# TUI-NICR/EMSANet

Hardware: AMD Instinct MI355X
Metric: images/sec (640x480 RGB-D, bs=32/GPU) fwd+bwd (higher is better)
Workload: dtype f32; 1 GPU; BASELINE.json configs[1]: full EMSANet RGB-D (resnet34-NBt1D x2, SE-add fusion, PPM, semantic+instance+orientation+scene heads), 640x480, bs=32/GPU, f32, train mode (BN batch stats, Dropout2d), step = fwd + bwd (fixed output cotangents) + grad all-reduce + SGD-nesterov update at lr 0 (fixed weights) replayed from a hipGraph; global_batch=32, parallelism=dp1, weights=random init (deterministic), mode=train-hipgraph

## Files before the change

emsanet_amd/csrc/conv_mfma.hip:

```cpp
#include "common.h"

#include <type_traits>
#include <vector>

#include "prof.h"

namespace {

struct ProfSlotImpl {
  hipEvent_t a, b;
  int cls;
  double flops, bytes;
};
std::vector<ProfSlotImpl> g_prof_pool;
size_t g_prof_used = 0;
int g_prof_every = 0;
int g_prof_seen[kProfClasses] = {0};
double g_prof_next_flops = 0.0;
const char* const kProfNames[kProfClasses] = {
    "conv_igemm_kernel<128,128,2,2>", "conv_igemm_kernel<128,64,4,2>",
    "conv_igemm_kernel<64,64,2,2>",   "conv_igemm_kernel<128,32,4,1>",
    "conv_wgrad_kernel<64,32,7,2,1,2>", "conv_wgrad_kernel<128,128,1,2,2,1> (unused)",
    "conv_wgrad_kernel<64,64,1,2,2,1>", "conv_wgrad_kernel<64,64,3,2,2,1>|conv_wgrad1d_wino_kernel<64,64> (1-D convs)",
    "conv1d_wino_kernel (1-D 3x1/1x3 convs)", "conv_h_kernel (16-bit igemm)",
// ... 841 lines not shown

  if (s_begin < s_end) {
    load_regs(s_begin);
    store_lds();
  }
  __syncthreads();

  for (int s = s_begin; s < s_end; ++s) {
    const bool has_next = s + 1 < s_end;
    mleft = mleft_n;
    mright = mright_n;
    if (has_next) load_regs(s + 1);
    const float* d = dS + lh * BCO + wco * 32 + l31;
    const float* x = xS + lh * BCI + wci * 32 + l31;
#pragma unroll
    for (int kk = 0; kk < PK / 2; ++kk) {
      const int r = 2 * kk + lh;
      const float fa = d[kk * 2 * BCO];
      const bool okl = !((mleft >> r) & 1u), okr = !((mright >> r) & 1u);
#pragma unroll
      for (int t = 0; t < 3; ++t) {
        float fb = x[(kk * 2 + t) * BCI];
        if (t == 0) fb = okl ? fb : 0.f;
        if (t == 2) fb = okr ? fb : 0.f;
        acc[0][t] = __builtin_amdgcn_mfma_f32_32x32x2f32(fa, fb, acc[0][t], 0, 0, 0);
      }
    }
    __syncthreads();
    if (has_next) store_lds();
    __syncthreads();
  }

  if (p.ws != nullptr) {
    float* wt = p.ws + (((size_t)ks * p.R + kr) * p.n_tiles + tile) * (3 * BCO * BCI);
#pragma unroll
    for (int t = 0; t < 3; ++t)
#pragma unroll
      for (int r = 0; r < 16; ++r) {
        const int row = (r & 3) + 8 * (r >> 2) + 4 * lh;
        wt[(t * BCO + wco * 32 + row) * BCI + wci * 32 + l31] = acc[0][t][r];
      }
  } else {
#pragma unroll
  for (int t = 0; t < 3; ++t)
#pragma unroll
    for (int q = 0; q < NQ; ++q) {
      const int ci = ci0 + wci * 32 + l31;
#pragma unroll
      for (int r = 0; r < 16; ++r) {
        const int row = (r & 3) + 8 * (r >> 2) + 4 * lh;
        const int co = co0 + wco * 32 + row;
#if EMSA_ABL & 2
        if (co < p.n_ch && ci < p.k_ch && acc[q][t][r] == 1.2345e30f)
#else
        if (co < p.n_ch && ci < p.k_ch)
#endif
          unsafeAtomicAdd(p.dw + ((size_t)(kr * 3 + t) * p.n_ch + co) * p.k_ch + ci, acc[q][t][r]);
      }
    }
  }
  if (do_bias) {
    float* red = smem;
    __syncthreads();
    red[d_r * BCO + d_c4 + 0] = bsum.x;
    red[d_r * BCO + d_c4 + 1] = bsum.y;
    red[d_r * BCO + d_c4 + 2] = bsum.z;
    red[d_r * BCO + d_c4 + 3] = bsum.w;
    __syncthreads();
    if (tid < BCO) {
      float a = 0.f;
      for (int r = 0; r < 256 / DTPR; ++r) a += red[r * BCO + tid];
      if (p.ws_bias != nullptr)
        p.ws_bias[((size_t)ks * p.n_co_tiles + co_t) * BCO + tid] = a;
      else if (co0 + tid < p.n_ch)
        unsafeAtomicAdd(p.dbias + co0 + tid, a);
    }
  }
}

typedef __bf16 gbf16x8 __attribute__((ext_vector_type(8)));
#ifndef EMSA_W1DW_XBN_WPE
#define EMSA_W1DW_XBN_WPE 3
#endif
template <int BCO, int BCI, bool BF16 = false, typename T = float, bool XBN = false>
__global__ __launch_bounds__(256, XBN ? EMSA_W1DW_XBN_WPE : EMSA_W1DW_WPE) void conv_wgrad1d_wino_kernel(const Wgrad1dArgs p) {
  static_assert(BCO == 64 && BCI == 64, "wave layout below is for a 64x64 (co x ci) tile");
  static_assert(!XBN || (!BF16 && sizeof(T) == 4), "the folded input BatchNorm is an fp32 form");
  constexpr uint32_t ES = sizeof(T);
  constexpr int PK = 32, NP = PK / 2, XROWS = PK + 2;
  extern __shared__ __attribute__((aligned(16))) float smem[];
  float* const eS = smem;
  float* const dS = smem + NP * 4 * BCO;
  constexpr int kBL = 20;
  __bf16* const eH = reinterpret_cast<__bf16*>(smem);
  __bf16* const dH = eH + 4 * BCO * kBL;

  const int tid = threadIdx.x, lane = tid & 63, wave = tid >> 6;
  const int l31 = lane & 31, lh = lane >> 5;
  const int wco = wave & 1, wci = wave >> 1;
#if EMSA_W1D_XCD
  const int wg = emsa_xcd_remap(blockIdx.x, gridDim.x);
#else
  const int wg = blockIdx.x;
#endif
  const int tile = wg % p.n_tiles, kr = (wg / p.n_tiles) % p.R;
  const int ks = wg / (p.n_tiles * p.R);
  const int dline = p.R == 3 ? kr - 1 : 0;
  const int ci_t = tile % p.n_ci_tiles, co_t = tile / p.n_ci_tiles;
  const int co0 = co_t * BCO, ci0 = ci_t * BCI;
  const int s_begin = ks * p.steps_per_split;
  const int s_end = min(s_begin + p.steps_per_split, p.steps_total);
  const __amdgpu_buffer_rsrc_t rs_in = make_rsrc(p.in, p.in_bytes);
  const __amdgpu_buffer_rsrc_t rs_dy = make_rsrc(p.dout, p.dout_bytes);
  const int col4 = (tid & 15) * 4, pr = tid >> 4;
  const bool do_bias = p.dbias != nullptr && ci_t == 0 && kr == 0;
  const bool dok = co0 + col4 < p.n_ch, xok = ci0 + col4 < p.k_ch;
  const uint32_t dadd = dok ? (uint32_t)(co0 + col4) * ES : 0u, dmask = dok ? 0u : kOOB;
  const uint32_t xadd = xok ? (uint32_t)(ci0 + col4) * ES : 0u, xmask = xok ? 0u : kOOB;

  typename Raw4<T>::type re_raw[2], rx_raw[4];
  float4 bsum = emsa_zero4();
  uint32_t x_real = 0;
  float* const xbnS = smem + NP * 4 * (BCO + BCI);
  if constexpr (XBN) {
    if (tid < 2 * BCI) {
      const int ch = ci0 + (tid & (BCI - 1));
      const float* src = tid < BCI ? p.in_scale : p.in_shift;
      xbnS[tid] = ch < p.k_ch ? src[ch] : 0.f;
    }
  }
  auto load_regs = [&](int s) {
    const int k = s * PK + lane - 1;
    const bool valid = lane < XROWS && k >= 0 && k < p.M;
    const uint32_t ku = valid ? (uint32_t)k : 0u;
    const uint32_t img = fast_div(ku, p.div_al);
    const uint32_t line = fast_div(ku, p.div_l);
    const int b_ = (int)(ku - __umul24(line, (uint32_t)p.L));
    const int a_ = (int)(line - __umul24(img, (uint32_t)p.A));
    const int a2 = a_ + dline;
    const bool in_line = valid && b_ < p.Lr;
    const uint32_t off_d = in_line
        ? (__umul24(img, (uint32_t)p.dy_simg) + __umul24((uint32_t)a_, (uint32_t)p.dy_sa) +
           __umul24((uint32_t)b_, (uint32_t)p.dy_sb)) * ES : kOOB;
    const uint32_t off_x = (in_line && a2 >= 0 && a2 < p.A)
        ? (__umul24(img, (uint32_t)p.in_simg) + __umul24((uint32_t)a2, (uint32_t)p.in_sa) +
           __umul24((uint32_t)b_, (uint32_t)p.in_sb)) * ES : kOOB;
    const uint32_t off_xl = b_ == p.L - 1 ? kOOB : off_x;
    const uint32_t off_xr = b_ == 0 ? kOOB : off_x;
    const int l0 = (2 * pr) * 4;
    const uint32_t o_e0 = (uint32_t)__builtin_amdgcn_ds_bpermute(l0 + 4, (int)off_d);
    const uint32_t o_e1 = (uint32_t)__builtin_amdgcn_ds_bpermute(l0 + 8, (int)off_d);
    const uint32_t o_d0 = (uint32_t)__builtin_amdgcn_ds_bpermute(l0, (int)off_xl);
    const uint32_t o_d1 = (uint32_t)__builtin_amdgcn_ds_bpermute(l0 + 4, (int)off_x);
    const uint32_t o_d2 = (uint32_t)__builtin_amdgcn_ds_bpermute(l0 + 8, (int)off_x);
    const uint32_t o_d3 = (uint32_t)__builtin_amdgcn_ds_bpermute(l0 + 12, (int)off_xr);
    re_raw[0] = buf_ld4raw<T>(rs_dy, (o_e0 + dadd) | dmask);
    re_raw[1] = buf_ld4raw<T>(rs_dy, (o_e1 + dadd) | dmask);
    rx_raw[0] = buf_ld4raw<T>(rs_in, (o_d0 + xadd) | xmask);
    rx_raw[1] = buf_ld4raw<T>(rs_in, (o_d1 + xadd) | xmask);
    rx_raw[2] = buf_ld4raw<T>(rs_in, (o_d2 + xadd) | xmask);
    rx_raw[3] = buf_ld4raw<T>(rs_in, (o_d3 + xadd) | xmask);
    if constexpr (XBN)
      x_real = (~o_d0 >> 31) | ((~o_d1 >> 31) << 1) | ((~o_d2 >> 31) << 2) | ((~o_d3 >> 31) << 3);
  };
  auto add4 = [](const float4& a, const float4& b) {
    return make_float4(a.x + b.x, a.y + b.y, a.z + b.z, a.w + b.w);
  };
  auto sub4 = [](const float4& a, const float4& b) {
    return make_float4(a.x - b.x, a.y - b.y, a.z - b.z, a.w - b.w);
  };
  auto store_lds = [&]() {
    const float4 re[2] = {raw_f4(re_raw[0], (T*)nullptr), raw_f4(re_raw[1], (T*)nullptr)};
    float4 rx[4] = {raw_f4(rx_raw[0], (T*)nullptr), raw_f4(rx_raw[1], (T*)nullptr),
                    raw_f4(rx_raw[2], (T*)nullptr), raw_f4(rx_raw[3], (T*)nullptr)};
    if constexpr (XBN) {
      typedef float f2 __attribute__((ext_vector_type(2)));
      const float4 sc = emsa_ld4(xbnS + col4), sh = emsa_ld4(xbnS + BCI + col4);
#pragma unroll
      for (int r = 0; r < 4; ++r) {
        const float cap = (x_real >> r) & 1u ? __builtin_inff() : 0.f;
        const f2 lo = __builtin_elementwise_fma(f2{rx[r].x, rx[r].y}, f2{sc.x, sc.y}, f2{sh.x, sh.y});
        const f2 hi = __builtin_elementwise_fma(f2{rx[r].z, rx[r].w}, f2{sc.z, sc.w}, f2{sh.z, sh.w});
        rx[r] = make_float4(__builtin_amdgcn_fmed3f(lo.x, 0.f, cap), __builtin_amdgcn_fmed3f(lo.y, 0.f, cap),
                            __builtin_amdgcn_fmed3f(hi.x, 0.f, cap), __builtin_amdgcn_fmed3f(hi.y, 0.f, cap));
      }
    }
// ... 46 lines not shown
  for (int s = s_begin; s < s_end; ++s) {
#endif
    const bool has_next = s + 1 < s_end;
    if (has_next) load_regs(s + 1);
    if constexpr (BF16) {
#pragma unroll
      for (int c = 0; c < 4; ++c) {
        const uint2* ea = reinterpret_cast<const uint2*>(eH + (c * BCO + wco * 32 + l31) * kBL + 8 * lh);
        const uint2* da = reinterpret_cast<const uint2*>(dH + (c * BCI + wci * 32 + l31) * kBL + 8 * lh);
        const uint2 e0 = ea[0], e1 = ea[1], d0 = da[0], d1 = da[1];
        const uint4 eu = make_uint4(e0.x, e0.y, e1.x, e1.y), du = make_uint4(d0.x, d0.y, d1.x, d1.y);
        acc[c] = __builtin_amdgcn_mfma_f32_32x32x16_bf16(__builtin_bit_cast(gbf16x8, eu),
                                                         __builtin_bit_cast(gbf16x8, du), acc[c],
                                                         0, 0, 0);
      }
    } else {
    const float* e = eS + lh * 4 * BCO + wco * 32 + l31;
    const float* d = dS + lh * 4 * BCI + wci * 32 + l31;
#pragma unroll
    for (int kk = 0; kk < NP / 2; ++kk) {
#pragma unroll
      for (int c = 0; c < 4; ++c)
        acc[c] = __builtin_amdgcn_mfma_f32_32x32x2f32(e[(kk * 8 + c) * BCO], d[(kk * 8 + c) * BCI],
                                                      acc[c], 0, 0, 0);
    }
    }
    __syncthreads();
    if (has_next) store_lds();
    __syncthreads();
  }

#pragma unroll
  for (int r = 0; r < 16; ++r) {
    const float m0 = acc[0][r], m1 = acc[1][r], m2 = acc[2][r], m3 = acc[3][r];
    const float hs = 0.5f * (m1 + m2);
    acc[0][r] = m0 + hs;
    acc[1][r] = 0.5f * (m1 - m2);
    acc[2][r] = hs - m3;
  }

  if (p.ws != nullptr) {
    float* wt = p.ws + (((size_t)ks * p.R + kr) * p.n_tiles + tile) * (3 * BCO * BCI);
#pragma unroll
    for (int t = 0; t < 3; ++t)
#pragma unroll
      for (int r = 0; r < 16; ++r) {
        const int row = (r & 3) + 8 * (r >> 2) + 4 * lh;
        wt[(t * BCO + wco * 32 + row) * BCI + wci * 32 + l31] = acc[t][r];
      }
  } else {
    const int ci = ci0 + wci * 32 + l31;
#pragma unroll
    for (int t = 0; t < 3; ++t)
#pragma unroll
      for (int r = 0; r < 16; ++r) {
        const int row = (r & 3) + 8 * (r >> 2) + 4 * lh;
        const int co = co0 + wco * 32 + row;
#if EMSA_ABL & 2
        if (co < p.n_ch && ci < p.k_ch && acc[t][r] == 1.2345e30f)
#else
        if (co < p.n_ch && ci < p.k_ch)
#endif
          unsafeAtomicAdd(p.dw + ((size_t)(kr * 3 + t) * p.n_ch + co) * p.k_ch + ci, acc[t][r]);
      }
  }
  if (do_bias) {
    float* red = smem;
    __syncthreads();
    red[pr * BCO + col4 + 0] = bsum.x;
    red[pr * BCO + col4 + 1] = bsum.y;
    red[pr * BCO + col4 + 2] = bsum.z;
    red[pr * BCO + col4 + 3] = bsum.w;
    __syncthreads();
    if (tid < BCO) {
      float a = 0.f;
      for (int r = 0; r < NP; ++r) a += red[r * BCO + tid];
      if (p.ws_bias != nullptr)
        p.ws_bias[((size_t)ks * p.n_co_tiles + co_t) * BCO + tid] = a;
      else if (co0 + tid < p.n_ch)
        unsafeAtomicAdd(p.dbias + co0 + tid, a);
    }
  }
}

#ifndef EMSA_WH_DBG
#define EMSA_WH_DBG 0
#endif
#if EMSA_WH_DBG
__device__ long long g_wh_dbg[8 * 4 * 4096];
#define WH_MARK(ph)                                               \
  do {                                                            \
    const long long t_ = (long long)__builtin_readcyclecounter(); \
    dbg_t[ph] += t_ - dbg_prev;                                   \
    dbg_prev = t_;                                                \
  } while (0)
#else
#define WH_MARK(ph) do {} while (0)
#endif
#if defined(__HIP_DEVICE_COMPILE__)
#define EMSA_NO_LSOPT __attribute__((target("no-load-store-opt")))
#else
#define EMSA_NO_LSOPT
#endif
#ifndef EMSA_WH_PK
#define EMSA_WH_PK 64
#endif
constexpr int kWH_PK = EMSA_WH_PK;
constexpr int kWH_NH = kWH_PK / 64;
constexpr int kWH_ROW = kWH_PK + 4;
template <typename T, int MODE = 0>
__global__ __launch_bounds__(256, 3) EMSA_NO_LSOPT void conv_wgrad1d_h_kernel(const Wgrad1dArgs p) {
  constexpr int BCO = 64, BCI = 64;
  constexpr uint32_t ES = sizeof(T);
  constexpr int NT_ = MODE == 1 ? 1 : 3;
  typedef unsigned int u32x4h __attribute__((ext_vector_type(4)));
  extern __shared__ __attribute__((aligned(16))) float smem[];
  T* const dS = reinterpret_cast<T*>(smem);
  T* const xS = dS + BCO * kWH_ROW;
  T* const oS = xS + BCI * kWH_ROW;

  const int tid = threadIdx.x, lane = tid & 63, wave = __builtin_amdgcn_readfirstlane(tid >> 6);
  const int l31 = lane & 31, lh = lane >> 5;
  const int wco = wave & 1, wci = wave >> 1;
#if EMSA_W1D_XCD
  const int wg = emsa_xcd_remap(blockIdx.x, gridDim.x);
#else
  const int wg = blockIdx.x;
#endif
  const int tile = wg % p.n_tiles, kr = (wg / p.n_tiles) % p.R;
  const int ks = wg / (p.n_tiles * p.R);
  const int dline = kr * p.dl_mul + p.dl_off;
  const int ci_t = tile % p.n_ci_tiles, co_t = tile / p.n_ci_tiles;
  const int co0 = co_t * BCO, ci0 = ci_t * BCI;
  const int s_begin = ks * p.steps_per_split;
  const int s_end = min(s_begin + p.steps_per_split, p.steps_total);
  const __amdgpu_buffer_rsrc_t rs_in = make_rsrc(p.in, p.in_bytes);
  const __amdgpu_buffer_rsrc_t rs_dy = make_rsrc(p.dout, p.dout_bytes);
  const int q = (lane & 3) | ((lane >> 4) << 2);
  const int pg = wave * 4 + ((lane >> 2) & 3);
  const bool do_bias = p.dbias != nullptr && ci_t == 0 && kr == 0;
  const bool dok = co0 + 4 * q < p.n_ch, xok = ci0 + 4 * q < p.k_ch;
  const uint32_t dadd = dok ? (uint32_t)(co0 + 4 * q) * ES : 0u, dmask = dok ? 0u : kOOB;
  const uint32_t xadd = xok ? (uint32_t)(ci0 + 4 * q) * ES : 0u, xmask = xok ? 0u : kOOB;

  uint32_t oo_last = kOOB;
  auto px_off = [&](int k, uint32_t& od, uint32_t& ox) {
    const bool valid = k >= 0 && k < p.M;
    const uint32_t ku = valid ? (uint32_t)k : 0u;
    const uint32_t img = fast_div(ku, p.div_al);
    const uint32_t line = fast_div(ku, p.div_l);
    const int b_ = (int)(ku - __umul24(line, (uint32_t)p.L));
    const int a_ = (int)(line - __umul24(img, (uint32_t)p.A));
    const int a2 = a_ * p.x_mul_a + dline;
    const bool in_line = valid && b_ < p.Lr;
    od = in_line ? (__umul24(img, (uint32_t)p.dy_simg) + __umul24((uint32_t)a_, (uint32_t)p.dy_sa) +
                    __umul24((uint32_t)b_, (uint32_t)p.dy_sb)) * ES : kOOB;
    ox = (in_line && a2 >= 0 && a2 < p.in_Ax)
        ? (__umul24(img, (uint32_t)p.in_simg) + __umul24((uint32_t)a2, (uint32_t)p.in_sa1) +
           __umul24((uint32_t)b_, (uint32_t)p.in_sb)) * ES : kOOB;
    if constexpr (MODE == 2)
      oo_last = (ox != kOOB && 2 * b_ + 1 < p.in_Lx) ? ox + (uint32_t)p.in_sb1 * ES : kOOB;
  };

  u32x2w rd[kWH_NH][4], rx[kWH_NH][4], ro[kWH_NH][4];
  u32x2w sv_d = {0u, 0u}, sv_x = {0u, 0u}, sv_o = {0u, 0u};
  float4 bsum = emsa_zero4();
// ... 134 lines not shown
    if constexpr (MODE != 1) prev_s = *reinterpret_cast<const unsigned*>(srow0 + kWH_PK);
    if constexpr (MODE == 0) prev_d = *reinterpret_cast<const unsigned*>(drow0 + kWH_PK);
    __builtin_amdgcn_s_setprio(1);
#pragma unroll
    for (int k16 = 0; k16 < kWH_PK / 16; ++k16) {
      const u32x4h a = ld8(drow, 16 * k16);
      const u32x4h c = ld8(xrow, 16 * k16);
      const ev8 av = __builtin_bit_cast(ev8, a);
      if constexpr (MODE == 1) {
        mma(acc[0], av, c);
      } else if constexpr (MODE == 2) {
        const u32x4h o_ = ld8(srow, 16 * k16);
        const u32x4h lft = shifted(o_, prev_s);
        mma(acc[0], av, lft);
        mma(acc[1], av, c);
        mma(acc[2], av, o_);
      } else {
        const u32x4h lft = shifted(c, prev_s);
        const u32x4h a_sh = shifted(a, prev_d);
        mma(acc[0], av, lft);
        mma(acc[1], av, c);
        mma(acc[2], __builtin_bit_cast(ev8, a_sh), c);
      }
    }
    __builtin_amdgcn_s_setprio(0);
    WH_MARK(1);
    __syncthreads();
    WH_MARK(2);
    if (has_next) store_lds();
    WH_MARK(3);
    __syncthreads();
    WH_MARK(4);
  }

  if (p.ws != nullptr) {
    float* wt = p.ws + (((size_t)ks * p.R + kr) * p.n_tiles + tile) * (NT_ * BCO * BCI);
#pragma unroll
    for (int t = 0; t < NT_; ++t)
#pragma unroll
      for (int r = 0; r < 16; ++r) {
        const int row = (r & 3) + 8 * (r >> 2) + 4 * lh;
        wt[(t * BCO + wco * 32 + row) * BCI + wci * 32 + l31] = acc[t][r];
      }
  } else {
    const int ci = ci0 + wci * 32 + l31;
#pragma unroll
    for (int t = 0; t < NT_; ++t)
#pragma unroll
      for (int r = 0; r < 16; ++r) {
        const int row = (r & 3) + 8 * (r >> 2) + 4 * lh;
        const int co = co0 + wco * 32 + row;
        if (co < p.n_ch && ci < p.k_ch)
          unsafeAtomicAdd(p.dw + ((size_t)(kr * NT_ + t) * p.n_ch + co) * p.k_ch + ci, acc[t][r]);
      }
  }
#if EMSA_WH_DBG
  WH_MARK(6);
  dbg_t[7] = dbg_prev - dbg_t0;
  if (lane == 0 && blockIdx.x < 4096)
    for (int i = 0; i < 8; ++i) g_wh_dbg[(blockIdx.x * 4 + wave) * 8 + i] = dbg_t[i];
#endif
  if (do_bias) {
    float* red = smem;
    __syncthreads();
    red[pg * BCO + 4 * q + 0] = bsum.x;
    red[pg * BCO + 4 * q + 1] = bsum.y;
    red[pg * BCO + 4 * q + 2] = bsum.z;
    red[pg * BCO + 4 * q + 3] = bsum.w;
    __syncthreads();
    if (tid < BCO) {
      float a = 0.f;
      for (int r = 0; r < 16; ++r) a += red[r * BCO + tid];
      if (p.ws_bias != nullptr)
        p.ws_bias[((size_t)ks * p.n_co_tiles + co_t) * BCO + tid] = a;
      else if (co0 + tid < p.n_ch)
        unsafeAtomicAdd(p.dbias + co0 + tid, a);
    }
  }
}

constexpr int kWT_PK = 64;
constexpr int kWT_RS = 96;
constexpr int kWT_IMG = (kWT_PK + 2) * kWT_RS;
constexpr int kWgradMultiMax = 4;
struct WgradMulti {
  Wgrad1dArgs j[kWgradMultiMax];
};

template <typename T, bool XBN = false>
__device__ __forceinline__ void wgrad1d_tr_body(const Wgrad1dArgs& p, const int bid, const int nblk) {
  constexpr int BCO = 64, BCI = 64;
  constexpr uint32_t ES = sizeof(T);
  typedef unsigned int u32x4h __attribute__((ext_vector_type(4)));
  typedef short s16x4 __attribute__((ext_vector_type(4)));
  typedef __attribute__((address_space(3))) s16x4 lds_s16x4;
  extern __shared__ __attribute__((aligned(16))) float smem[];
  T* const dS = reinterpret_cast<T*>(smem);
  T* const xS = dS + kWT_IMG;
  float* const xbnS = reinterpret_cast<float*>(xS + kWT_IMG);

  const int tid = threadIdx.x, lane = tid & 63, wave = __builtin_amdgcn_readfirstlane(tid >> 6);
  const int wco = wave & 1, wci = wave >> 1;
#if EMSA_W1D_XCD
  const int wg = emsa_xcd_remap(bid, nblk);
#else
  const int wg = bid;
#endif
  const int tile = wg % p.n_tiles, kr = (wg / p.n_tiles) % p.R;
  const int ks = wg / (p.n_tiles * p.R);
  const int dline = kr * p.dl_mul + p.dl_off;
  const int ci_t = tile % p.n_ci_tiles, co_t = tile / p.n_ci_tiles;
  const int co0 = co_t * BCO, ci0 = ci_t * BCI;
  const int s_begin = ks * p.steps_per_split;
  const int s_end = min(s_begin + p.steps_per_split, p.steps_total);
  const __amdgpu_buffer_rsrc_t rs_in = make_rsrc(p.in, p.in_bytes);
  const __amdgpu_buffer_rsrc_t rs_dy = make_rsrc(p.dout, p.dout_bytes);
  const int lp = tid >> 2, ch0 = (lane & 3) * 8;
  const bool do_bias = p.dbias != nullptr && ci_t == 0 && kr == 0;
  uint32_t dadd[2], xadd[2];
#pragma unroll
  for (int h = 0; h < 2; ++h) {
    dadd[h] = co0 + ch0 + 32 * h < p.n_ch ? (uint32_t)(co0 + ch0 + 32 * h) * ES : kOOB;
    xadd[h] = ci0 + ch0 + 32 * h < p.k_ch ? (uint32_t)(ci0 + ch0 + 32 * h) * ES : kOOB;
  }
  auto px_off = [&](int k, uint32_t& od, uint32_t& ox) {
    const bool valid = k >= 0 && k < p.M;
    const uint32_t ku = valid ? (uint32_t)k : 0u;
    const uint32_t img = fast_div(ku, p.div_al);
    const uint32_t line = fast_div(ku, p.div_l);
    const int b_ = (int)(ku - __umul24(line, (uint32_t)p.L));
    const int a_ = (int)(line - __umul24(img, (uint32_t)p.A));
    const int a2 = a_ * p.x_mul_a + dline;
    const bool in_line = valid && b_ < p.Lr;
    od = in_line ? (__umul24(img, (uint32_t)p.dy_simg) + __umul24((uint32_t)a_, (uint32_t)p.dy_sa) +
                    __umul24((uint32_t)b_, (uint32_t)p.dy_sb)) * ES : kOOB;
    ox = (in_line && a2 >= 0 && a2 < p.in_Ax)
        ? (__umul24(img, (uint32_t)p.in_simg) + __umul24((uint32_t)a2, (uint32_t)p.in_sa1) +
           __umul24((uint32_t)b_, (uint32_t)p.in_sb)) * ES : kOOB;
  };
  const bool xbn = XBN && p.in_scale != nullptr;
  if constexpr (XBN) {
    if (xbn && tid < 2 * BCI) {
      const int ch = ci0 + (tid & (BCI - 1));
      const float* src = tid < BCI ? p.in_scale : p.in_shift;
      xbnS[tid] = ch < p.k_ch ? src[ch] : 0.f;
    }
  }
  u32x4h rd[2], rx[2];
  [[maybe_unused]] bool x_real = false;
  auto load_px = [&](int k, u32x4h (&d)[2], u32x4h (&x)[2]) {
    uint32_t od, ox;
    px_off(k, od, ox);
    if constexpr (XBN) x_real = ox != kOOB;
#pragma unroll
    for (int h = 0; h < 2; ++h) {
      d[h] = __builtin_amdgcn_raw_buffer_load_b128(rs_dy, (int)(od | dadd[h]) >= 0 ? (int)(od + dadd[h]) : (int)kOOB, 0, 0);
      x[h] = __builtin_amdgcn_raw_buffer_load_b128(rs_in, (int)(ox | xadd[h]) >= 0 ? (int)(ox + xadd[h]) : (int)kOOB, 0, 0);
    }
  };
  float bsum[2][8];
#pragma unroll
  for (int h = 0; h < 2; ++h)
#pragma unroll
    for (int e = 0; e < 8; ++e) bsum[h][e] = 0.f;
  [[maybe_unused]] auto xbn_apply = [&](u32x4h (&x)[2]) {
    if constexpr (XBN) {
      if (xbn) {
        typedef typename std::conditional<std::is_same<T, emsa_f16>::value, _Float16, __bf16>::type EX;
        typedef EX ex8 __attribute__((ext_vector_type(8)));
        typedef float fx8 __attribute__((ext_vector_type(8)));
// ... 692 lines not shown
          } else
            hipLaunchKernelGGL((conv_wgrad1d_tr_kernel<T>), grid, dim3(256),
                               (size_t)2 * kWT_IMG * sizeof(T), st, w);
        } else if (in_scale) {
          prof_end(ps, st);
          return EMSA_E_SHAPE;
        } else
          hipLaunchKernelGGL((conv_wgrad1d_h_kernel<T, 0>), grid, dim3(256),
                             (size_t)2 * 64 * kWH_ROW * sizeof(T), st, w);
      } else if constexpr (!kF16)
      hipLaunchKernelGGL((conv_wgrad1d_wino_kernel<BCO, BCI, true, T>),
                         dim3(w.n_tiles * w.R * pl.ksplit), dim3(256),
                         (size_t)(16 * 4 * (BCO + BCI)) * sizeof(float), st, w);
    } else if (pl.wino && in_scale) {
      if constexpr (!kHalf)
        hipLaunchKernelGGL((conv_wgrad1d_wino_kernel<BCO, BCI, false, float, true>),
                           dim3(w.n_tiles * w.R * pl.ksplit), dim3(256),
                           (size_t)(16 * 4 * (BCO + BCI) + 2 * BCI) * sizeof(float), st, w);
    } else if (in_scale) {
      prof_end(ps, st);
      return EMSA_E_SHAPE;
    } else if (pl.wino && bf16)
      hipLaunchKernelGGL((conv_wgrad1d_wino_kernel<BCO, BCI, true>),
                         dim3(w.n_tiles * w.R * pl.ksplit), dim3(256),
                         (size_t)(16 * 4 * (BCO + BCI)) * sizeof(float), st, w);
    else if (pl.wino)
      hipLaunchKernelGGL((conv_wgrad1d_wino_kernel<BCO, BCI>), dim3(w.n_tiles * w.R * pl.ksplit),
                         dim3(256), (size_t)(16 * 4 * (BCO + BCI)) * sizeof(float), st, w);
    else
      hipLaunchKernelGGL((conv_wgrad1d_kernel<BCO, BCI>), dim3(w.n_tiles * w.R * pl.ksplit),
                         dim3(256), lds, st, w);
    static const bool rows_on = [] {
      const char* e = getenv("EMSA_WGRAD_REDUCE_ROWS");
      return !(e && e[0] == '0');
    }();
    if (ws != nullptr && rows_on && pl.ksplit <= 16 && w.n_tiles >= 32)
      hipLaunchKernelGGL(wgrad1d_reduce_rows_kernel, dim3(w.n_tiles * 4 + w.n_co_tiles),
                         dim3(256), 0, st, ws, w.ws_bias, pl.ksplit, w.n_tiles, w.n_ci_tiles,
                         w.n_co_tiles, w.n_ch, w.k_ch, w.R, dw, dbias, w.taps);
    else if (ws != nullptr)
      hipLaunchKernelGGL(wgrad1d_reduce_kernel, dim3(w.n_tiles * w.R * w.taps * 64 + w.n_co_tiles),
                         dim3(256), 0, st, ws, w.ws_bias, pl.ksplit, w.n_tiles, w.n_ci_tiles,
                         w.n_co_tiles, w.n_ch, w.k_ch, w.R, dw, dbias, w.taps);
    prof_end(ps, st);
    return emsa_launch_status();
  }
  if (in_scale) return EMSA_E_SHAPE;
  if (taps == 7 && g->k_ch <= 32) return launch_wgrad<64, 32, 7, 2, 1, 2, T>(a, st);
  if (taps == 2 && g->k_ch <= 32) return launch_wgrad<64, 32, 2, 2, 1, 2, T>(a, st);
  if (taps == 1) {
    return launch_wgrad<64, 64, 1, 2, 2, 1, T>(a, st);
  }
  return launch_wgrad<64, 64, 3, 2, 2, 1, T>(a, st);
}
}

extern "C" int emsa_conv_wgrad(const EmsaConvGeom* g, const float* in, const float* dout,
                               float* dw, float* dbias, float* ws, void* stream) {
  return conv_wgrad_impl<float>(g, in, dout, dw, dbias, ws, stream);
}

extern "C" int emsa_conv_wgrad_inbn(const EmsaConvGeom* g, const float* in, const float* dout,
                                    float* dw, float* dbias, float* ws, const float* in_scale,
                                    const float* in_shift, void* stream) {
  if (!in_scale || !in_shift) return EMSA_E_ARG;
  return conv_wgrad_impl<float>(g, in, dout, dw, dbias, ws, stream, in_scale, in_shift);
}

extern "C" int emsa_conv_wgrad_t(int32_t dtype, const EmsaConvGeom* g, const void* in,
                                 const void* dout, float* dw, float* dbias, float* ws,
                                 void* stream) {
  if (dtype == EMSA_DT_F32)
    return conv_wgrad_impl<float>(g, (const float*)in, (const float*)dout, dw, dbias, ws, stream);
  if (dtype == EMSA_DT_BF16)
    return conv_wgrad_impl<emsa_bf16>(g, (const emsa_bf16*)in, (const emsa_bf16*)dout, dw, dbias,
                                      ws, stream);
  if (dtype == EMSA_DT_F16)
    return conv_wgrad_impl<emsa_f16>(g, (const emsa_f16*)in, (const emsa_f16*)dout, dw, dbias,
                                     ws, stream);
  return EMSA_E_ARG;
}

namespace {
bool plan_wgrad_multi(int n_jobs, const EmsaConvGeom* geoms, Wgrad1dPlan* pls, int& ksplit) {
  if (n_jobs < 2 || n_jobs > kWgradMultiMax || !wgrad16_tr()) return false;
  for (int j = 0; j < n_jobs; ++j) {
    const EmsaConvGeom* g = geoms + j;
    if (!geom_ok(g) || geom_mapped(g) || g->div_h != 1 || g->div_w != 1) return false;
    if (!direct16_geom(g) || !plan_wgrad1d(g, dout_is_aligned(g, nullptr), pls[j], 2, true)) return false;
    if (pls[j].mode != 0) return false;
    if ((g->k_ch & 7) || (g->n_ch & 7) || (g->ld_out & 7) || (g->in_px_stride & 7) ||
        (g->in_row_stride & 7) || (g->in_img_stride & 7))
      return false;
    if (pls[j].w.n_tiles != pls[0].w.n_tiles || pls[j].w.R != pls[0].w.R ||
        pls[j].w.n_ch != pls[0].w.n_ch || pls[j].w.k_ch != pls[0].w.k_ch)
      return false;
  }
  const Wgrad1dArgs& w0 = pls[0].w;
  static const int budget = [] {
    const char* e = getenv("EMSA_WGRAD_MULTI_WGS");
    const int v = e ? atoi(e) : 0;
    return v >= 64 ? v : 768;
  }();
  int ks = budget / (n_jobs * w0.n_tiles * w0.R);
  for (int j = 0; j < n_jobs; ++j) {
    const int max_split = (pls[j].w.steps_total + 3) / 4;
    if (ks > max_split) ks = max_split;
  }
  if (ks < 1) ks = 1;
  int n_split = 0;
  for (int j = 0; j < n_jobs; ++j) {
    Wgrad1dArgs& w = pls[j].w;
    w.steps_per_split = (w.steps_total + ks - 1) / ks;
    const int need = (w.steps_total + w.steps_per_split - 1) / w.steps_per_split;
    if (need > n_split) n_split = need;
  }
  ksplit = n_split;
  for (int j = 0; j < n_jobs; ++j) pls[j].ksplit = n_split;
  return true;
}
int64_t wgrad_multi_job_floats(const Wgrad1dPlan& pl) {
  return (int64_t)pl.ksplit * ((int64_t)pl.w.n_tiles * pl.w.R * pl.w.taps * 4096 + (int64_t)pl.w.n_co_tiles * 64);
}
}

extern "C" int64_t emsa_conv_wgrad_multi_ws_bytes(int32_t dtype, int32_t n_jobs, const EmsaConvGeom* geoms) {
  if (dtype != EMSA_DT_BF16 || !geoms) return 0;
  Wgrad1dPlan pls[kWgradMultiMax];
  int ks = 0;
  if (!plan_wgrad_multi(n_jobs, geoms, pls, ks)) return 0;
  int64_t fl = 0;
  for (int j = 0; j < n_jobs; ++j) fl += wgrad_multi_job_floats(pls[j]);
  return fl * (int64_t)sizeof(float);
}

namespace {
int conv_wgrad_multi_impl(int32_t dtype, int32_t n_jobs, const EmsaConvGeom* geoms,
                          const void* const* in, const void* const* dout, float* const* dw,
                          float* const* dbias, float* ws, const float* const* in_scale,
                          const float* const* in_shift, void* stream) {
  if (dtype != EMSA_DT_BF16) return EMSA_E_ARG;
  if (!geoms || !in || !dout || !dw || !dbias || !ws) return EMSA_E_ARG;
  Wgrad1dPlan pls[kWgradMultiMax];
  int ks = 0;
  if (!plan_wgrad_multi(n_jobs, geoms, pls, ks)) return EMSA_E_SHAPE;
  hipStream_t st = (hipStream_t)stream;
  WgradMulti m;
  ReduceMulti r;
  float* wsp = ws;
  double flops = 0.0, bytes = 0.0;
  bool any_xbn = false;
  for (int j = 0; j < kWgradMultiMax; ++j) {
    const int k = j < n_jobs ? j : 0;
    if (j < n_jobs) {
      const EmsaConvGeom* g = geoms + j;
      if (!in[j] || !dout[j] || !dw[j]) return EMSA_E_ARG;
      if ((((uintptr_t)in[j]) | ((uintptr_t)dout[j])) & 15) return EMSA_E_SHAPE;
      Wgrad1dArgs& w = pls[j].w;
      w.in = reinterpret_cast<const float*>(in[j]);
      w.dout = reinterpret_cast<const float*>(dout[j]);
      w.dw = dw[j];
      w.dbias = dbias[j];
      w.ws = wsp;
      w.ws_bias = wsp + (size_t)ks * w.n_tiles * w.R * w.taps * 4096;
      w.in_scale = in_scale ? in_scale[j] : nullptr;
      w.in_shift = in_shift ? in_shift[j] : nullptr;
      if ((w.in_scale == nullptr) != (w.in_shift == nullptr)) return EMSA_E_ARG;
      any_xbn = any_xbn || w.in_scale != nullptr;
      wsp += wgrad_multi_job_floats(pls[j]);
      flops += algo_flops(*g);
      bytes += (double)g->n_img * g->in_h * g->in_w * g->k_ch * 2.0 +
               (double)g->n_img * g->out_h * g->out_w * g->n_ch * 2.0 + (double)g->kh * g->kw * g->n_ch * g->k_ch * 4.0;
    }
    m.j[j] = pls[k].w;
    r.ws[j] = pls[k].w.ws; r.ws_bias[j] = pls[k].w.ws_bias; r.dw[j] = pls[k].w.dw; r.dbias[j] = pls[k].w.dbias;
  }
  const Wgrad1dArgs& w0 = pls[0].w;
  r.splits = ks; r.n_tiles = w0.n_tiles; r.n_ci_tiles = w0.n_ci_tiles; r.n_co_tiles = w0.n_co_tiles;
  r.n_ch = w0.n_ch; r.k_ch = w0.k_ch; r.R = w0.R; r.taps = w0.taps;
  const int ps = prof_begin(kProfClassWgradH, flops, st, bytes);
  if (any_xbn)
    hipLaunchKernelGGL((conv_wgrad1d_tr_multi_kernel<emsa_bf16, true>), dim3(w0.n_tiles * w0.R * ks, n_jobs),
                       dim3(256), (size_t)2 * kWT_IMG * sizeof(emsa_bf16) + 2 * 64 * sizeof(float), st, m);
  else
    hipLaunchKernelGGL((conv_wgrad1d_tr_multi_kernel<emsa_bf16>), dim3(w0.n_tiles * w0.R * ks, n_jobs),
                       dim3(256), (size_t)2 * kWT_IMG * sizeof(emsa_bf16), st, m);
  if (ks <= 16 && w0.n_tiles >= 32)
    hipLaunchKernelGGL((wgrad1d_reduce_multi_kernel<true>), dim3(w0.n_tiles * 4 + w0.n_co_tiles, n_jobs),
                       dim3(256), 0, st, r);
  else
    hipLaunchKernelGGL((wgrad1d_reduce_multi_kernel<false>),
                       dim3(w0.n_tiles * w0.R * w0.taps * 64 + w0.n_co_tiles, n_jobs), dim3(256), 0, st, r);
  prof_end(ps, st);
  return emsa_launch_status();
}
}

extern "C" int emsa_conv_wgrad_multi_t(int32_t dtype, int32_t n_jobs, const EmsaConvGeom* geoms,
                                       const void* const* in, const void* const* dout,
                                       float* const* dw, float* const* dbias, float* ws,
                                       void* stream) {
  return conv_wgrad_multi_impl(dtype, n_jobs, geoms, in, dout, dw, dbias, ws, nullptr, nullptr, stream);
}

extern "C" int emsa_conv_wgrad_multi_inbn_t(int32_t dtype, int32_t n_jobs, const EmsaConvGeom* geoms,
                                            const void* const* in, const void* const* dout,
                                            float* const* dw, float* const* dbias, float* ws,
                                            const float* const* in_scale,
                                            const float* const* in_shift, void* stream) {
  if (!in_scale || !in_shift) return EMSA_E_ARG;
  return conv_wgrad_multi_impl(dtype, n_jobs, geoms, in, dout, dw, dbias, ws, in_scale, in_shift, stream);
}

extern "C" int emsa_conv_wgrad_inbn_t(int32_t dtype, const EmsaConvGeom* g, const void* in,
                                      const void* dout, float* dw, float* dbias, float* ws,
                                      const float* in_scale, const float* in_shift, void* stream) {
  if (!in_scale || !in_shift) return EMSA_E_ARG;
  if (dtype == EMSA_DT_F32)
    return conv_wgrad_impl<float>(g, (const float*)in, (const float*)dout, dw, dbias, ws, stream,
                                  in_scale, in_shift);
  if (dtype == EMSA_DT_BF16)
    return conv_wgrad_impl<emsa_bf16>(g, (const emsa_bf16*)in, (const emsa_bf16*)dout, dw, dbias,
                                      ws, stream, in_scale, in_shift);
  return EMSA_E_ARG;
}

extern "C" int emsa_prof_enable(int32_t every) {
  g_prof_every = every > 0 ? every : 0;
  return EMSA_OK;
}
extern "C" int emsa_prof_next_flops(double flops) {
  g_prof_next_flops = g_prof_every > 0 ? flops : 0.0;
  return EMSA_OK;
}
extern "C" int emsa_prof_reset(void) {
  g_prof_used = 0;
  for (int i = 0; i < kProfClasses; ++i) g_prof_seen[i] = 0;
  return EMSA_OK;
}
extern "C" int emsa_prof_seen(int32_t cls) { return (cls >= 0 && cls < kProfClasses) ? g_prof_seen[cls] : 0; }
extern "C" const char* emsa_prof_name(int32_t cls) {
  return (cls >= 0 && cls < kProfClasses) ? kProfNames[cls] : "";
}
extern "C" int emsa_prof_read_bytes(int32_t cls, double* total_bytes) {
  if (!total_bytes) return EMSA_E_ARG;
  double b = 0.0;
  for (size_t i = 0; i < g_prof_used; ++i)
    if (g_prof_pool[i].cls == cls) b += g_prof_pool[i].bytes;
  *total_bytes = b;
  return EMSA_OK;
}
extern "C" int emsa_prof_read(int32_t cls, double* total_ms, double* total_flops,
                              int32_t* launches) {
  if (!total_ms || !total_flops || !launches) return EMSA_E_ARG;
  double ms = 0.0, fl = 0.0;
  int n = 0;
  for (size_t i = 0; i < g_prof_used; ++i) {
    const ProfSlotImpl& s = g_prof_pool[i];
    if (s.cls != cls) continue;
    float t = 0.f;
    if (hipEventElapsedTime(&t, s.a, s.b) != hipSuccess) return EMSA_E_LAUNCH;
    ms += t;
    fl += s.flops;
    ++n;
  }
  *total_ms = ms;
  *total_flops = fl;
  *launches = n;
  return EMSA_OK;
}
// ... 1 lines not shown
```

emsanet_amd/functional.py:

```python
import ctypes
import os

import torch

from . import _lib
from ._lib import EmsaConvGeom, check

ACT_NONE, ACT_RELU = 0, 1


def _stream():
    return torch.cuda.current_stream().cuda_stream


_POISON = bool(os.environ.get('EMSA_POISON'))


def _empty(shape, device, dtype=torch.float32):
    t = torch.empty(shape, device=device, dtype=dtype)
    if _POISON:
        t.fill_(float('nan') if dtype.is_floating_point else 111)
    return t


# ... 809 lines not shown
def wgrad_wino2d_selected(spec):
    if not wino2d_eligible(spec) or _BF16_MFMA:
        return False
    if WGRAD_WINO2D is not None:
        return bool(WGRAD_WINO2D)
    if _WGRAD_WINO2D_ENV is not None:
        return _WGRAD_WINO2D_ENV != '0'
    return (spec.cin, spec.cout) in WGRAD_WINO2D_SHAPES


def _conv_wgrad_wino2d(x, dy, spec, g, want_bias, like, dw_out, db_out):
    global WGRAD_WINO2D_FALLBACKS
    L = _lib.lib()
    ws_bytes = L.emsa_conv_wgrad_wino2d_ws_bytes(0, g) if L.emsa_conv_wgrad_wino2d_supported(0, g) else 0
    if ws_bytes <= 0:
        WGRAD_WINO2D_FALLBACKS += 1
        return None
    nw = 9 * spec.cout * spec.cin
    ws = _empty((ws_bytes // 4,), x.device)
    if like is not None and dw_out is not None and (db_out is not None or not want_bias):
        dw, db = dw_out.view(-1), db_out
    else:
        buf = _empty((nw + (spec.cout if want_bias else 0),), x.device)
        dw = buf[:nw]
        db = buf[nw:] if want_bias else None
    packed = like is None
    check(L.emsa_conv_wgrad_wino2d(0, g, _p(x), _p(dy), _p(dw), _p(db), _p(ws), 1 if packed else 0,
                                   _stream()), 'emsa_conv_wgrad_wino2d')
    if packed:
        return dw, db, True
    return dw.view(like.shape), db, False


def conv_wgrad(x, dy, spec, want_bias, like=None, two_pass=None, dw_out=None, db_out=None,
               in_affine=None):
    if two_pass is None:
        two_pass = deterministic_wgrad()
    n, c, h, w = x.shape
    g = spec.geom_fwd(n, h, w, ld_of(x), ld_of(dy))
    if (in_affine is None and x.dtype == torch.float32 and dy.dtype == torch.float32 and
            two_pass is not False and wgrad_wino2d_selected(spec)):
        res = _conv_wgrad_wino2d(x, dy, spec, g, want_bias, like, dw_out, db_out)
        if res is not None:
            return res
    L = _lib.lib()
    taps = spec.kh * spec.kw
    nw = taps * spec.cout * spec.cin
    nb = spec.cout if want_bias else 0
    ws_bytes = call_t('emsa_conv_wgrad_ws_bytes', dt(x), g) if (like is not None and two_pass) else 0
    if ws_bytes > 0:
        ws = _empty((ws_bytes // 4,), x.device)
        if dw_out is not None and (db_out is not None or not want_bias):
            dw, db = dw_out.view(-1), db_out
        else:
            buf = _empty((nw + nb,), x.device)
            dw = buf[:nw]
            db = buf[nw:] if want_bias else None
    else:
        buf = _zeros((nw + nb,), x.device)
        ws = None
        dw = buf[:nw]
        db = buf[nw:] if want_bias else None
    if x.dtype != dy.dtype:
        raise _lib.EmsaError(f"weight gradient of {x.dtype} activations with a {dy.dtype} gradient")
    if in_affine is not None and dt(x) != 0:
        if ws is None:
            raise _lib.EmsaError("in_affine (16-bit): the two-pass weight gradient only")
        check(L.emsa_conv_wgrad_inbn_t(dt(x), g, _p(x), _p(dy), _p(dw), _p(db), _p(ws),
                                       _p(in_affine[0]), _p(in_affine[1]), _stream()),
              'emsa_conv_wgrad_inbn_t')
    elif in_affine is not None:
        check(L.emsa_conv_wgrad_inbn(g, _p(x), _p(dy), _p(dw), _p(db), _p(ws), _p(in_affine[0]),
                                     _p(in_affine[1]), _stream()), 'emsa_conv_wgrad_inbn')
    else:
        check(call_t('emsa_conv_wgrad', dt(x), g, _p(x), _p(dy), _p(dw), _p(db), _p(ws), _stream()),
              'emsa_conv_wgrad')
    if ws is not None:
        return dw.view(like.shape), db, False
    return dw, db, True


WGRAD_MULTI = os.environ.get('EMSA_WGRAD_MULTI', '1') != '0'
WGRAD_MULTI_MAX = 4


def wgrad_multi_eligible(x, spec):
    return (WGRAD_MULTI and x.dtype == torch.bfloat16 and deterministic_wgrad() and spec.sh == 1 and
            spec.sw == 1 and (spec.kh, spec.kw, spec.ph, spec.pw) in ((3, 1, 1, 0), (1, 3, 0, 1)) and
            spec.cin % 8 == 0 and spec.cout % 8 == 0)


def conv_wgrad_multi(jobs):
    n_jobs = len(jobs)
    if n_jobs < 2 or n_jobs > WGRAD_MULTI_MAX:
        return None
    L = _lib.lib()
    geoms = (_lib.EmsaConvGeom * n_jobs)()
    for j, (x, dy, spec, *_rest) in enumerate(jobs):
        n, c, h, w = x.shape
        if x.dtype != dy.dtype:
            raise _lib.EmsaError(f"weight gradient of {x.dtype} activations with a {dy.dtype} gradient")
        g = spec.geom_fwd(n, h, w, ld_of(x), ld_of(dy))
        ctypes.memmove(ctypes.byref(geoms[j]), ctypes.byref(g), ctypes.sizeof(_lib.EmsaConvGeom))
    code = dt(jobs[0][0])
    ws_bytes = L.emsa_conv_wgrad_multi_ws_bytes(code, n_jobs, geoms)
    if ws_bytes <= 0:
        return None
    dev = jobs[0][0].device
    ws = _empty((ws_bytes // 4,), dev)
    arr = lambda: (ctypes.c_void_p * n_jobs)()
    a_in, a_dy, a_dw, a_db, a_sc, a_sh = arr(), arr(), arr(), arr(), arr(), arr()
    outs = []
    any_aff = False
    for j, (x, dy, spec, like, dw_out, db_out, want_bias, *aff) in enumerate(jobs):
        if aff and aff[0] is not None:
            a_sc[j], a_sh[j] = _p(aff[0][0]), _p(aff[0][1])
            any_aff = True
        nw = spec.kh * spec.kw * spec.cout * spec.cin
        if dw_out is not None and (db_out is not None or not want_bias):
            dw, db = dw_out.view(-1), db_out
        else:
            buf = _empty((nw + (spec.cout if want_bias else 0),), dev)
            dw = buf[:nw]
            db = buf[nw:] if want_bias else None
        a_in[j], a_dy[j], a_dw[j], a_db[j] = _p(x), _p(dy), _p(dw), _p(db)
        outs.append((dw.view(like.shape), db))
    if any_aff:
        check(L.emsa_conv_wgrad_multi_inbn_t(code, n_jobs, geoms, a_in, a_dy, a_dw, a_db, _p(ws), a_sc,
                                             a_sh, _stream()), 'emsa_conv_wgrad_multi_inbn_t')
    else:
        check(L.emsa_conv_wgrad_multi_t(code, n_jobs, geoms, a_in, a_dy, a_dw, a_db, _p(ws), _stream()),
              'emsa_conv_wgrad_multi_t')
    return outs


STEM_ROWS = os.environ.get('EMSA_STEM_ROWS', '1') != '0'


class StemSpec:

    def __init__(self, cin, cout=64):
        self.cin, self.cout = cin, cout
        self.rows = cin == 1 and STEM_ROWS
        self.taps = 2 if self.rows else 7
        self._geoms = {}

    def out_hw(self, h, w):
        return (h + 6 - 7) // 2 + 1, (w + 6 - 7) // 2 + 1

    def geom(self, n, h, w, ld_out):
        key = (n, h, w, ld_out)
        g = self._geoms.get(key)
        if g is None:
            oh, ow = self.out_hw(h, w)
            wp = w + 8
            if self.rows:
                hp = h + 4
                g = EmsaConvGeom(n, hp, wp, oh, ow, 32, self.cout, 2, 1,
                                 2, 0, 4, 1, 2, 0, 1, 1,
                                 hp * wp * 4, wp * 4, 4, ld_out)
            else:
                g = EmsaConvGeom(n, h, wp, oh, ow, 32, self.cout, 7, 1,
                                 2, -3, 1, 1, 2, 0, 1, 1,
                                 h * wp * 4, wp * 4, 4, ld_out)
            self._geoms[key] = g
        return g


def stem_pack_input(x_nchw, dtype=torch.float32):
    x = x_nchw.contiguous()
    n, c, h, w = x.shape
    if c == 1 and STEM_ROWS:
        xp = _empty((n, h + 4, w + 8, 4), x.device, dtype)
        check(_lib.lib().emsa_stem_pack_input_rows_t(DT[dtype], _p(x), _p(xp), n, h, w, _stream()),
              'emsa_stem_pack_input_rows_t')
        return xp
    xp = _empty((n, h, w + 8, 4), x.device, dtype)
    check(call_t('emsa_stem_pack_input', DT[dtype], _p(x), _p(xp), n, c, h, w, _stream()),
          'emsa_stem_pack_input')
    return xp


def stem_pack_weight(w, dtype=torch.float32):
    cout, cin = w.shape[:2]
    if cin == 1 and STEM_ROWS:
        wp = _empty(2 * cout * 32, w.device, dtype)
        check(_lib.lib().emsa_stem_pack_weight_rows_t(DT[dtype], _p(w), _p(wp), cout, _stream()),
              'emsa_stem_pack_weight_rows_t')
        return wp
# ... 616 lines not shown
```

Measured before the change: 350.9 images/s.

## Batch fp32 1-D Winograd weight-gradient convs into one multi-job launch

Moves the fp32 1-D Winograd weight-gradient kernel body into a device function and adds a multi-job kernel that handles up to four same-shape 3x1/1x3 wgrad jobs in a single grid using blockIdx.y. The multi-wgrad planner, workspace sizing and Python eligibility check are extended to fp32 inputs, gated by a minimum activation size and 64-channel alignment. The intent is to cut kernel launch count and fill the GPU better for the small 1-D convs in the NBt1D blocks. The cost is an extra eligibility path that can fall back, plus a fixed split count shared across all jobs in a batch.

```diff
diff --git a/emsanet_amd/csrc/conv_mfma.hip b/emsanet_amd/csrc/conv_mfma.hip
--- a/emsanet_amd/csrc/conv_mfma.hip
+++ b/emsanet_amd/csrc/conv_mfma.hip
@@ -947,8 +947,12 @@
 #ifndef EMSA_W1DW_XBN_WPE
 #define EMSA_W1DW_XBN_WPE 3
 #endif
+constexpr int kWgradMultiMax = 4;
+struct WgradMulti {
+  Wgrad1dArgs j[kWgradMultiMax];
+};
 template <int BCO, int BCI, bool BF16 = false, typename T = float, bool XBN = false>
-__global__ __launch_bounds__(256, XBN ? EMSA_W1DW_XBN_WPE : EMSA_W1DW_WPE) void conv_wgrad1d_wino_kernel(const Wgrad1dArgs p) {
+__device__ __forceinline__ void wgrad1d_wino_body(const Wgrad1dArgs& p, const int bid, const int nblk) {
   static_assert(BCO == 64 && BCI == 64, "wave layout below is for a 64x64 (co x ci) tile");
   static_assert(!XBN || (!BF16 && sizeof(T) == 4), "the folded input BatchNorm is an fp32 form");
   constexpr uint32_t ES = sizeof(T);
@@ -964,9 +968,9 @@
   const int l31 = lane & 31, lh = lane >> 5;
   const int wco = wave & 1, wci = wave >> 1;
 #if EMSA_W1D_XCD
-  const int wg = emsa_xcd_remap(blockIdx.x, gridDim.x);
+  const int wg = emsa_xcd_remap(bid, nblk);
 #else
-  const int wg = blockIdx.x;
+  const int wg = bid;
 #endif
   const int tile = wg % p.n_tiles, kr = (wg / p.n_tiles) % p.R;
   const int ks = wg / (p.n_tiles * p.R);
@@ -1179,6 +1183,14 @@
     }
   }
 }
+template <int BCO, int BCI, bool BF16 = false, typename T = float, bool XBN = false>
+__global__ __launch_bounds__(256, XBN ? EMSA_W1DW_XBN_WPE : EMSA_W1DW_WPE) void conv_wgrad1d_wino_kernel(const Wgrad1dArgs p) {
+  wgrad1d_wino_body<BCO, BCI, BF16, T, XBN>(p, blockIdx.x, gridDim.x);
+}
+template <int BCO, int BCI>
+__global__ __launch_bounds__(256, EMSA_W1DW_WPE) void conv_wgrad1d_wino_multi_kernel(const WgradMulti m) {
+  wgrad1d_wino_body<BCO, BCI>(m.j[blockIdx.y], blockIdx.x, gridDim.x);
+}
 
 #ifndef EMSA_WH_DBG
 #define EMSA_WH_DBG 0
@@ -1479,10 +1491,6 @@
 constexpr int kWT_PK = 64;
 constexpr int kWT_RS = 96;
 constexpr int kWT_IMG = (kWT_PK + 2) * kWT_RS;
-constexpr int kWgradMultiMax = 4;
-struct WgradMulti {
-  Wgrad1dArgs j[kWgradMultiMax];
-};
 
 template <typename T, bool XBN = false>
 __device__ __forceinline__ void wgrad1d_tr_body(const Wgrad1dArgs& p, const int bid, const int nblk) {
@@ -2341,16 +2349,33 @@
 }
 
 namespace {
-bool plan_wgrad_multi(int n_jobs, const EmsaConvGeom* geoms, Wgrad1dPlan* pls, int& ksplit) {
-  if (n_jobs < 2 || n_jobs > kWgradMultiMax || !wgrad16_tr()) return false;
+bool wgrad_bf16_mfma() {
+  static const bool v = [] {
+    const char* e = getenv("EMSA_BF16_MFMA");
+    return e && e[0] == '1';
+  }();
+  return v;
+}
+bool plan_wgrad_multi(bool f32, int n_jobs, const EmsaConvGeom* geoms, Wgrad1dPlan* pls, int& ksplit) {
+  if (n_jobs < 2 || n_jobs > kWgradMultiMax) return false;
+  if (f32 ? wgrad_bf16_mfma() : !wgrad16_tr()) return false;
+  const int min_steps = f32 ? 8 : 4;
   for (int j = 0; j < n_jobs; ++j) {
     const EmsaConvGeom* g = geoms + j;
     if (!geom_ok(g) || geom_mapped(g) || g->div_h != 1 || g->div_w != 1) return false;
-    if (!direct16_geom(g) || !plan_wgrad1d(g, dout_is_aligned(g, nullptr), pls[j], 2, true)) return false;
+    if (f32) {
+      if (!plan_wgrad1d(g, dout_is_aligned(g, nullptr), pls[j]) || !pls[j].wino || pls[j].w.R != 1)
+        return false;
+      if ((g->k_ch & 63) || (g->n_ch & 63) || (g->in_px_stride & 3) || (g->in_row_stride & 3) ||
+          (g->in_img_stride & 3))
+        return false;
+    } else {
+      if (!direct16_geom(g) || !plan_wgrad1d(g, dout_is_aligned(g, nullptr), pls[j], 2, true)) return false;
+      if ((g->k_ch & 7) || (g->n_ch & 7) || (g->ld_out & 7) || (g->in_px_stride & 7) ||
+          (g->in_row_stride & 7) || (g->in_img_stride & 7))
+        return false;
+    }
     if (pls[j].mode != 0) return false;
-    if ((g->k_ch & 7) || (g->n_ch & 7) || (g->ld_out & 7) || (g->in_px_stride & 7) ||
-        (g->in_row_stride & 7) || (g->in_img_stride & 7))
-      return false;
     if (pls[j].w.n_tiles != pls[0].w.n_tiles || pls[j].w.R != pls[0].w.R ||
         pls[j].w.n_ch != pls[0].w.n_ch || pls[j].w.k_ch != pls[0].w.k_ch)
       return false;
@@ -2363,7 +2388,7 @@
   }();
   int ks = budget / (n_jobs * w0.n_tiles * w0.R);
   for (int j = 0; j < n_jobs; ++j) {
-    const int max_split = (pls[j].w.steps_total + 3) / 4;
+    const int max_split = (pls[j].w.steps_total + min_steps - 1) / min_steps;
     if (ks > max_split) ks = max_split;
   }
   if (ks < 1) ks = 1;
@@ -2384,10 +2409,10 @@
 }
 
 extern "C" int64_t emsa_conv_wgrad_multi_ws_bytes(int32_t dtype, int32_t n_jobs, const EmsaConvGeom* geoms) {
-  if (dtype != EMSA_DT_BF16 || !geoms) return 0;
+  if ((dtype != EMSA_DT_BF16 && dtype != EMSA_DT_F32) || !geoms) return 0;
   Wgrad1dPlan pls[kWgradMultiMax];
   int ks = 0;
-  if (!plan_wgrad_multi(n_jobs, geoms, pls, ks)) return 0;
+  if (!plan_wgrad_multi(dtype == EMSA_DT_F32, n_jobs, geoms, pls, ks)) return 0;
   int64_t fl = 0;
   for (int j = 0; j < n_jobs; ++j) fl += wgrad_multi_job_floats(pls[j]);
   return fl * (int64_t)sizeof(float);
@@ -2398,11 +2423,14 @@
                           const void* const* in, const void* const* dout, float* const* dw,
                           float* const* dbias, float* ws, const float* const* in_scale,
                           const float* const* in_shift, void* stream) {
-  if (dtype != EMSA_DT_BF16) return EMSA_E_ARG;
+  const bool f32 = dtype == EMSA_DT_F32;
+  if (dtype != EMSA_DT_BF16 && !f32) return EMSA_E_ARG;
   if (!geoms || !in || !dout || !dw || !dbias || !ws) return EMSA_E_ARG;
+  if (f32 && (in_scale || in_shift)) return EMSA_E_SHAPE;
+  const double esize = f32 ? 4.0 : 2.0;
   Wgrad1dPlan pls[kWgradMultiMax];
   int ks = 0;
-  if (!plan_wgrad_multi(n_jobs, geoms, pls, ks)) return EMSA_E_SHAPE;
+  if (!plan_wgrad_multi(f32, n_jobs, geoms, pls, ks)) return EMSA_E_SHAPE;
   hipStream_t st = (hipStream_t)stream;
   WgradMulti m;
   ReduceMulti r;
@@ -2428,8 +2456,8 @@
       any_xbn = any_xbn || w.in_scale != nullptr;
       wsp += wgrad_multi_job_floats(pls[j]);
       flops += algo_flops(*g);
-      bytes += (double)g->n_img * g->in_h * g->in_w * g->k_ch * 2.0 +
-               (double)g->n_img * g->out_h * g->out_w * g->n_ch * 2.0 + (double)g->kh * g->kw * g->n_ch * g->k_ch * 4.0;
+      bytes += (double)g->n_img * g->in_h * g->in_w * g->k_ch * esize +
+               (double)g->n_img * g->out_h * g->out_w * g->n_ch * esize + (double)g->kh * g->kw * g->n_ch * g->k_ch * 4.0;
     }
     m.j[j] = pls[k].w;
     r.ws[j] = pls[k].w.ws; r.ws_bias[j] = pls[k].w.ws_bias; r.dw[j] = pls[k].w.dw; r.dbias[j] = pls[k].w.dbias;
@@ -2437,14 +2465,21 @@
   const Wgrad1dArgs& w0 = pls[0].w;
   r.splits = ks; r.n_tiles = w0.n_tiles; r.n_ci_tiles = w0.n_ci_tiles; r.n_co_tiles = w0.n_co_tiles;
   r.n_ch = w0.n_ch; r.k_ch = w0.k_ch; r.R = w0.R; r.taps = w0.taps;
-  const int ps = prof_begin(kProfClassWgradH, flops, st, bytes);
-  if (any_xbn)
+  const int ps = prof_begin(f32 ? 7 : kProfClassWgradH, flops, st, bytes);
+  static const bool rows_on = [] {
+    const char* e = getenv("EMSA_WGRAD_REDUCE_ROWS");
+    return !(e && e[0] == '0');
+  }();
+  if (f32)
+    hipLaunchKernelGGL((conv_wgrad1d_wino_multi_kernel<64, 64>), dim3(w0.n_tiles * w0.R * ks, n_jobs),
+                       dim3(256), (size_t)(16 * 4 * (64 + 64)) * sizeof(float), st, m);
+  else if (any_xbn)
     hipLaunchKernelGGL((conv_wgrad1d_tr_multi_kernel<emsa_bf16, true>), dim3(w0.n_tiles * w0.R * ks, n_jobs),
                        dim3(256), (size_t)2 * kWT_IMG * sizeof(emsa_bf16) + 2 * 64 * sizeof(float), st, m);
   else
     hipLaunchKernelGGL((conv_wgrad1d_tr_multi_kernel<emsa_bf16>), dim3(w0.n_tiles * w0.R * ks, n_jobs),
                        dim3(256), (size_t)2 * kWT_IMG * sizeof(emsa_bf16), st, m);
-  if (ks <= 16 && w0.n_tiles >= 32)
+  if ((rows_on || !f32) && ks <= 16 && w0.n_tiles >= 32)
     hipLaunchKernelGGL((wgrad1d_reduce_multi_kernel<true>), dim3(w0.n_tiles * 4 + w0.n_co_tiles, n_jobs),
                        dim3(256), 0, st, r);
   else
diff --git a/emsanet_amd/functional.py b/emsanet_amd/functional.py
--- a/emsanet_amd/functional.py
+++ b/emsanet_amd/functional.py
@@ -915,12 +915,29 @@
 
 WGRAD_MULTI = os.environ.get('EMSA_WGRAD_MULTI', '1') != '0'
 WGRAD_MULTI_MAX = 4
+_WGRAD_MULTI32_ENV = os.environ.get('EMSA_WGRAD_MULTI32')
+_WGRAD_MULTI32_MIN_BYTES = int(float(os.environ.get('EMSA_WGRAD_MULTI32_MIN_MB', '8')) * (1 << 20))
+WGRAD_MULTI32 = None
+WGRAD_MULTI32_FALLBACKS = 0
+
+
+def _wgrad_multi32(x):
+    if _BF16_MFMA:
+        return False
+    if WGRAD_MULTI32 is not None:
+        return bool(WGRAD_MULTI32)
+    if _WGRAD_MULTI32_ENV is not None:
+        return _WGRAD_MULTI32_ENV != '0'
+    return x.numel() * 4 >= _WGRAD_MULTI32_MIN_BYTES
 
 
 def wgrad_multi_eligible(x, spec):
-    return (WGRAD_MULTI and x.dtype == torch.bfloat16 and deterministic_wgrad() and spec.sh == 1 and
-            spec.sw == 1 and (spec.kh, spec.kw, spec.ph, spec.pw) in ((3, 1, 1, 0), (1, 3, 0, 1)) and
-            spec.cin % 8 == 0 and spec.cout % 8 == 0)
+    if not (deterministic_wgrad() and spec.sh == 1 and spec.sw == 1 and
+            (spec.kh, spec.kw, spec.ph, spec.pw) in ((3, 1, 1, 0), (1, 3, 0, 1))):
+        return False
+    if x.dtype == torch.float32:
+        return spec.cin % 64 == 0 and spec.cout % 64 == 0 and _wgrad_multi32(x)
+    return WGRAD_MULTI and x.dtype == torch.bfloat16 and spec.cin % 8 == 0 and spec.cout % 8 == 0
 
 
 def conv_wgrad_multi(jobs):
@@ -936,8 +953,14 @@
         g = spec.geom_fwd(n, h, w, ld_of(x), ld_of(dy))
         ctypes.memmove(ctypes.byref(geoms[j]), ctypes.byref(g), ctypes.sizeof(_lib.EmsaConvGeom))
     code = dt(jobs[0][0])
+    if code == 0 and not all((len(job) < 8 or job[7] is None) and wgrad_multi_eligible(job[0], job[2])
+                             for job in jobs):
+        return None
     ws_bytes = L.emsa_conv_wgrad_multi_ws_bytes(code, n_jobs, geoms)
     if ws_bytes <= 0:
+        if code == 0:
+            global WGRAD_MULTI32_FALLBACKS
+            WGRAD_MULTI32_FALLBACKS += 1
         return None
     dev = jobs[0][0].device
     ws = _empty((ws_bytes // 4,), dev)
```

Result: no change. 351.0 images/s, median of 3 (+0.0%).
